# qinzheng93/GeoTransformer

Measured on NVIDIA H100. Metric: point-cloud pairs/sec (3DMatch-shape synth), higher is better.
Workload: dtype f32

## Files before the change

### geotransformer_b200/_lib.py

```python
import ctypes
import os
import threading

import torch

_HERE = os.path.dirname(os.path.abspath(__file__))
LIB_PATH = os.path.join(_HERE, 'libgeob200.so')
_lib = None

c_void_p, c_int64, c_int32, c_float, c_double, c_size_t, c_int = (
    ctypes.c_void_p, ctypes.c_int64, ctypes.c_int32, ctypes.c_float, ctypes.c_double, ctypes.c_size_t, ctypes.c_int)

SIGNATURES = {}


def _sig(name, restype, *argtypes):
    SIGNATURES[name] = (restype, list(argtypes))


P, I64, I32, F, D, SZ = c_void_p, c_int64, c_int32, c_float, c_double, c_size_t
_sig('geob200_last_error', ctypes.c_char_p)
_sig('geob200_launch_count', ctypes.c_uint64)
_sig('geob200_grid_subsample_workspace_bytes', SZ, I64, I64)
_sig('geob200_grid_subsample', c_int, P, I64, P, I64, F, P, P, P, SZ, P)
_sig('geob200_radius_search_workspace_bytes', SZ, I64, I64, I64)
_sig('geob200_radius_search', c_int, P, I64, P, I64, P, P, I64, F, I64, P, P, P, P, SZ, P)

_sig('geob200_neighbor_histogram', c_int, P, I64, I64, I64, I64, P, P)
_sig('geob200_kpconv_workspace_bytes', SZ, I64)
_sig('geob200_kpconv', c_int, P, P, P, P, I64, I64, I64, P, I64, P, P, I64, I64, F, P, P, SZ, P)
_sig('geob200_kpconv_tc_workspace_bytes', SZ, I64, I64, I64)
_sig('geob200_kpconv_tc', c_int, P, P, P, P, I64, I64, I64, P, I64, P, P, I64, I64, F, P, P, SZ, P)
_sig('geob200_set_linear_mode', None, c_int)
_sig('geob200_linear', c_int, P, I64, P, P, P, I64, I64, I64, I64, c_int, P)
_sig('geob200_split_tf32', c_int, P, I64, I64, I64, P, P)
_sig('geob200_linear_batched', c_int, P, I64, I64, P, I64, I64, P, I64, P, I64, I64, I64, I64, I64, I64, c_int, P)
_sig('geob200_group_norm_workspace_bytes', SZ, I64)
_sig('geob200_group_norm', c_int, P, I64, I64, I64, P, P, F, P, c_int, F, P, P, SZ, P)
_sig('geob200_fused_group_norm_workspace_bytes', SZ, I64, I64, I64)
_sig('geob200_linear_group_norm', c_int, P, I64, P, P, I64, I64, I64, I64, P, P, F, P, c_int, F, P, P, P, SZ, P)
_sig('geob200_kpconv_group_norm', c_int, P, P, P, P, I64, I64, I64, P, I64, P, P, I64, I64, F, I64, P, P, F, c_int, F, P, P, P, SZ,
     P, SZ, P)
_sig('geob200_group_norm_batched', c_int, P, I64, I64, I64, P, P, F, P, c_int, F, P, P, SZ, P, I64, P)
_sig('geob200_linear_group_norm_batched', c_int, P, I64, P, P, I64, I64, I64, I64, P, P, F, P, c_int, F, P, P, P, SZ, P, I64, P)
_sig('geob200_maxpool', c_int, P, P, I64, I64, I64, I64, P, P)
_sig('geob200_upsample_concat', c_int, P, P, I64, I64, P, I64, I64, I64, P, P)
_sig('geob200_point_to_node_partition_batched', c_int, P, P, I64, P, P, I64, P, P, P, P, P, P)
_sig('geob200_gather_rows', c_int, P, I64, I64, P, I64, P, P)
_sig('geob200_knn_partition', c_int, P, I64, P, I64, I64, P, P, P)
_sig('geob200_pairwise_distance', c_int, P, I64, P, I64, I64, c_int, P, P)
_sig('geob200_point_to_node_indices', c_int, P, I64, P, I64, P, P, P)
_sig('geob200_apply_transform', c_int, P, I64, P, P, P)
_sig('geob200_gse_indices_batched', c_int, P, I64, P, F, F, I64, P, P, P)
_sig('geob200_gse_embed_workspace_bytes', SZ, I64, I64)
_sig('geob200_gse_table_bytes', SZ, I64, I64, F, F)
_sig('geob200_gse_table_build', c_int, P, P, P, P, P, I64, I64, F, F, P, SZ, P)
_sig('geob200_gse_embed_table', c_int, P, P, I64, I64, P, SZ, I64, F, F, P, P, P, P, P, P, P)
_sig('geob200_gse_embed_pairs', c_int, P, P, I64, I64, P, P, P, P, P, P, P, P, c_int, P, SZ, P)
_sig('geob200_attention_workspace_bytes', SZ, I64, I64, I64)
_sig('geob200_attention', c_int, P, I64, P, I64, P, I64, P, P, P, I64, I64, I64, I64, P, I64, P, SZ, P)
_sig('geob200_set_attention_tma', c_int, c_int)
_sig('geob200_head_bias', c_int, P, I64, P, I64, I64, I64, P, P)
_sig('geob200_add_layernorm', c_int, P, P, P, P, I64, I64, F, P, P)
_sig('geob200_l2_normalize', c_int, P, I64, I64, P, P)
_sig('geob200_sinkhorn', c_int, P, P, P, P, I64, I64, I64, F, P, P)
# ... 128 lines not shown
```

### geotransformer_b200/csrc/kpconv.cu

```cuda
#include "common.cuh"
#include "geob200.h"

namespace geob200 {

constexpr int KP = 15;
constexpr int KP_PAD = 16;
constexpr int TQ = 32;
constexpr int CC = 32;

__device__ __forceinline__ void influence15(const float* __restrict__ kp_s, float rx, float ry, float rz, float inv_dummy,
                                            float sigma, float* w) {
#pragma unroll
    for (int k = 0; k < KP; ++k) {
        const float dx = rx - kp_s[3 * k], dy = ry - kp_s[3 * k + 1], dz = rz - kp_s[3 * k + 2];
        const float sq = __fadd_rn(__fadd_rn(__fmul_rn(dx, dx), __fmul_rn(dy, dy)), __fmul_rn(dz, dz));
        w[k] = fmaxf(1.0f - sqrtf(sq) / sigma, 0.0f);
    }
    (void)inv_dummy;
}

__global__ void __launch_bounds__(256) kpconv_c1_kernel(const float* __restrict__ feats, const float* __restrict__ q_pts,
                                                        const float* __restrict__ s_pts, const long long* __restrict__ nbr,
                                                        int H, const float* __restrict__ kp, const float* __restrict__ W,
                                                        const float* __restrict__ bias, float sigma, int Ns, int M, int Cout,
                                                        float* __restrict__ out) {
    __shared__ float kp_s[KP * 3];
    __shared__ float wk_s[16][KP_PAD];
    __shared__ float np_s[16];
    if (threadIdx.x < KP * 3) kp_s[threadIdx.x] = kp[threadIdx.x];
    __syncthreads();
    const int lane = threadIdx.x & 31, warp = threadIdx.x >> 5;
    const int sub = lane >> 4, sl = lane & 15;
    const int slot = warp * 2 + sub;
    const int m = blockIdx.x * 16 + slot;
    const bool live = m < M;
    float acc[KP];
#pragma unroll
    for (int k = 0; k < KP; ++k) acc[k] = 0.f;
    int npos = 0;
    if (live) {
        const float qx = q_pts[3ll * m], qy = q_pts[3ll * m + 1], qz = q_pts[3ll * m + 2];
        for (int h = sl; h < H; h += 16) {
            const long long idx = nbr[(long long)m * H + h];
            if (idx < Ns) {
                float w[KP];
                influence15(kp_s, s_pts[3 * idx] - qx, s_pts[3 * idx + 1] - qy, s_pts[3 * idx + 2] - qz, 0.f, sigma, w);
                const float f = feats[idx];
                npos += (f > 0.f);
#pragma unroll
                for (int k = 0; k < KP; ++k) acc[k] = fmaf(w[k], f, acc[k]);
// ... 4 lines not shown
    for (int k = 0; k < KP; ++k) {
#pragma unroll
        for (int o = 8; o > 0; o >>= 1) acc[k] += __shfl_xor_sync(0xffffffffu, acc[k], o);
    }
#pragma unroll
    for (int o = 8; o > 0; o >>= 1) npos += __shfl_xor_sync(0xffffffffu, npos, o);
    if (sl == 0) {
#pragma unroll
        for (int k = 0; k < KP; ++k) wk_s[slot][k] = acc[k];
        np_s[slot] = (float)max(npos, 1);
    }
    __syncwarp();
    if (!live) return;
    for (int c = sl; c < Cout; c += 16) {
        float o = 0.f;
#pragma unroll
        for (int k = 0; k < KP; ++k) o = fmaf(wk_s[slot][k], W[k * Cout + c], o);
        o = o / np_s[slot];
        if (bias != nullptr) o += bias[c];
        out[(long long)m * Cout + c] = o;
    }
}

__global__ void __launch_bounds__(256) row_positive_kernel(const float* __restrict__ x, int N, int C, unsigned char* __restrict__ pos) {
    const int lane = threadIdx.x & 31;
    const int n = blockIdx.x * 8 + (threadIdx.x >> 5);
    if (n >= N) return;
    float s = 0.f;
    for (int c = lane; c < C; c += 32) s += x[(long long)n * C + c];
    s = warp_sum(s);
    if (lane == 0) pos[n] = (s > 0.f) ? 1 : 0;
}

template <int CPL>
__global__ void __launch_bounds__(256, 4) kpconv_gather_kernel(const float* __restrict__ feats, const unsigned char* __restrict__ pos,
                                                            const float* __restrict__ q_pts, const float* __restrict__ s_pts,
                                                            const long long* __restrict__ nbr, int H, const float* __restrict__ kp,
                                                            float sigma, int Ns, int M, int Cin, float* __restrict__ wf,
                                                            float* __restrict__ inv_count) {
    __shared__ float infl[8][32][KP_PAD];
    __shared__ int sidx[8][32];
    __shared__ float kp_s[KP * 3];
    const int lane = threadIdx.x & 31, warp = threadIdx.x >> 5;
    if (threadIdx.x < KP * 3) kp_s[threadIdx.x] = kp[threadIdx.x];
    __syncthreads();
    const int m = blockIdx.x * 8 + warp;
    if (m >= M) return;
    const float qx = q_pts[3ll * m], qy = q_pts[3ll * m + 1], qz = q_pts[3ll * m + 2];
    int npos = 0;
    for (int c0 = 0; c0 < Cin; c0 += 32 * CPL) {
        float acc[CPL][KP];
#pragma unroll
        for (int p = 0; p < CPL; ++p)
#pragma unroll
            for (int k = 0; k < KP; ++k) acc[p][k] = 0.f;
        for (int h0 = 0; h0 < H; h0 += 32) {
            const int h = h0 + lane;
            const long long idx = (h < H) ? nbr[(long long)m * H + h] : (long long)Ns;
            float w[KP];
            int id = 0;
            if (idx < Ns) {
                id = (int)idx;
                influence15(kp_s, s_pts[3 * idx] - qx, s_pts[3 * idx + 1] - qy, s_pts[3 * idx + 2] - qz, 0.f, sigma, w);
                if (c0 == 0) npos += pos[idx];
            } else {
#pragma unroll
                for (int k = 0; k < KP; ++k) w[k] = 0.f;
            }
            __syncwarp();
#pragma unroll
            for (int k = 0; k < KP; ++k) infl[warp][lane][k] = w[k];
            infl[warp][lane][KP] = 0.f;
            sidx[warp][lane] = id;
            __syncwarp();
            const int hn = min(32, H - h0);
            for (int hb = 0; hb < hn; hb += 8) {
                float f[8][CPL];
#pragma unroll
                for (int u = 0; u < 8; ++u)
#pragma unroll
                    for (int p = 0; p < CPL; ++p)
                        f[u][p] = __ldg(feats + (long long)sidx[warp][(hb + u) & 31] * Cin + c0 + 32 * p + lane);
#pragma unroll
                for (int u = 0; u < 8; ++u) {
                    if (hb + u < hn) {
                        const float4* iv = reinterpret_cast<const float4*>(&infl[warp][hb + u][0]);
                        const float4 a0 = iv[0], a1 = iv[1], a2 = iv[2], a3 = iv[3];
                        const float wv[16] = {a0.x, a0.y, a0.z, a0.w, a1.x, a1.y, a1.z, a1.w, a2.x, a2.y, a2.z, a2.w, a3.x, a3.y, a3.z, a3.w};
#pragma unroll
                        for (int p = 0; p < CPL; ++p)
#pragma unroll
                            for (int k = 0; k < KP; ++k) acc[p][k] = fmaf(wv[k], f[u][p], acc[p][k]);
                    }
                }
            }
        }
#pragma unroll
        for (int p = 0; p < CPL; ++p) {
            float* wrow = wf + (long long)m * (KP * Cin) + c0 + 32 * p + lane;
#pragma unroll
            for (int k = 0; k < KP; ++k) wrow[(long long)k * Cin] = acc[p][k];
        }
    }
#pragma unroll
    for (int o = 16; o > 0; o >>= 1) npos += __shfl_xor_sync(0xffffffffu, npos, o);
    if (lane == 0) inv_count[m] = 1.0f / (float)max(npos, 1);
}

static void launch_kpconv_gather(const float* s_feats, const unsigned char* pos, const float* q_points, const float* s_points,
                                 const long long* neighbors, int n_neighbors, const float* kernel_points, float sigma, int n_support,
                                 int n_query, int c_in, float* wf, float* inv_count, cudaStream_t st) {
    const unsigned grid = (unsigned)((n_query + 7) / 8);
    if (c_in % 64 == 0)
        kpconv_gather_kernel<2><<<grid, 256, 0, st>>>(s_feats, pos, q_points, s_points, neighbors, n_neighbors, kernel_points, sigma,
                                                     n_support, n_query, c_in, wf, inv_count);
    else
        kpconv_gather_kernel<1><<<grid, 256, 0, st>>>(s_feats, pos, q_points, s_points, neighbors, n_neighbors, kernel_points, sigma,
                                                     n_support, n_query, c_in, wf, inv_count);
}

template <int RC>
__global__ void __launch_bounds__(256) kpconv_kernel(const float* __restrict__ feats, const unsigned char* __restrict__ pos,
                                                     const float* __restrict__ q_pts, const float* __restrict__ s_pts,
                                                     const long long* __restrict__ nbr, int H, const float* __restrict__ kp,
                                                     const float* __restrict__ W, const float* __restrict__ bias, float sigma,
                                                     int Ns, int M, int Cin, int Cout, float* __restrict__ out) {
    const int col0 = blockIdx.y * (RC * 32);
    extern __shared__ float smem[];
    float* wf = smem;
    float* infl = wf + TQ * KP * CC;
    int* sidx = (int*)(infl + 8 * 32 * KP_PAD);
    float* npos_s = (float*)(sidx + 8 * 32);
    float* kp_s = npos_s + TQ;
    const int lane = threadIdx.x & 31, warp = threadIdx.x >> 5;
    if (threadIdx.x < KP * 3) kp_s[threadIdx.x] = kp[threadIdx.x];
    __syncthreads();
    const int m0 = blockIdx.x * TQ;

    float acc_out[4][RC];
#pragma unroll
    for (int r = 0; r < 4; ++r)
#pragma unroll
        for (int j = 0; j < RC; ++j) acc_out[r][j] = 0.f;

    for (int c0 = 0; c0 < Cin; c0 += CC) {
        for (int q = warp; q < TQ; q += 8) {
            const int m = m0 + q;
            float acc[KP];
#pragma unroll
            for (int k = 0; k < KP; ++k) acc[k] = 0.f;
            int npos = 0;
// ... 594 lines not shown
            best = fmaxf(best, v);
        }
        y[(long long)m * C + c] = best;
    }
}

__global__ void __launch_bounds__(256) upsample_concat_kernel(const float* __restrict__ x, const long long* __restrict__ up,
                                                              int up_stride, int Ns, const float* __restrict__ skip, int M,
                                                              int C1, int C2, float* __restrict__ y) {
    const int lane = threadIdx.x & 31;
    const int m = blockIdx.x * 8 + (threadIdx.x >> 5);
    if (m >= M) return;
    const long long idx = up[(long long)m * up_stride];
    float* yr = y + (long long)m * (C1 + C2);
    for (int c = lane; c < C1; c += 32) yr[c] = (idx < Ns) ? x[idx * C1 + c] : 0.f;
    if (skip != nullptr)
        for (int c = lane; c < C2; c += 32) yr[C1 + c] = skip[(long long)m * C2 + c];
}

}

using namespace geob200;

namespace geob200 {
int linear_tc(const float* x, int64_t ldx, const float* w, int64_t ldw, const float* w_img, const float* bias, const float* row_scale, float* y, int64_t ldy,
              int64_t m, int64_t n, int64_t k, int relu, cudaStream_t st, const GnFuse* gn = nullptr);
static int g_linear_mode = 1;
}

extern "C" {

void geob200_set_linear_mode(int mode) { g_linear_mode = mode; }

size_t geob200_kpconv_workspace_bytes(int64_t n_support) { return (size_t)n_support + 256; }

size_t geob200_kpconv_tc_workspace_bytes(int64_t n_query, int64_t n_support, int64_t c_in) {
    return align_up((size_t)n_support, 256) + align_up((size_t)n_query * 4, 256) + (size_t)n_query * KP * (size_t)c_in * 4 + 1024;
}

int geob200_kpconv_tc(const float* s_feats, const float* q_points, const float* s_points, const int64_t* neighbors, int64_t n_query,
                      int64_t n_support, int64_t n_neighbors, const float* kernel_points, int64_t n_kernel, const float* weights_t,
                      const float* bias, int64_t c_in, int64_t c_out, float sigma, float* out, void* workspace, size_t workspace_bytes,
                      void* stream) {
    return geob200::kpconv_tc_impl(s_feats, q_points, s_points, neighbors, n_query, n_support, n_neighbors, kernel_points, n_kernel,
                                   weights_t, nullptr, bias, c_in, c_out, sigma, out, workspace, workspace_bytes, stream);
}
}

namespace geob200 {
int kpconv_tc_impl(const float* s_feats, const float* q_points, const float* s_points, const int64_t* neighbors, int64_t n_query,
                   int64_t n_support, int64_t n_neighbors, const float* kernel_points, int64_t n_kernel, const float* weights_t,
                   const float* w_img, const float* bias, int64_t c_in, int64_t c_out, float sigma, float* out, void* workspace,
                   size_t workspace_bytes, void* stream) {
    cudaStream_t st = (cudaStream_t)stream;
    GEOB_REQUIRE(n_kernel == KP, "kpconv_tc: kernel_size %lld unsupported", (long long)n_kernel);
    GEOB_REQUIRE(n_query > 0 && n_support > 0 && n_neighbors > 0, "kpconv_tc: empty input");
    GEOB_REQUIRE(c_in % 32 == 0 && c_out % 16 == 0 && c_out >= 32 && (c_out <= 128 || c_out % 128 == 0) && n_query >= 64,
                 "kpconv_tc: unsupported shape (%lld -> %lld, %lld queries)", (long long)c_in, (long long)c_out, (long long)n_query);
    GEOB_REQUIRE(workspace_bytes >= geob200_kpconv_tc_workspace_bytes(n_query, n_support, c_in), "kpconv_tc: workspace too small");
    Arena ar(workspace, workspace_bytes);
    unsigned char* pos = ar.take<unsigned char>(n_support);
    float* inv_count = ar.take<float>(n_query);
    float* wf = ar.take<float>((size_t)n_query * KP * c_in);
    row_positive_kernel<<<(unsigned)((n_support + 7) / 8), 256, 0, st>>>(s_feats, (int)n_support, (int)c_in, pos);
    launch_kpconv_gather(s_feats, pos, q_points, s_points, (const long long*)neighbors, (int)n_neighbors, kernel_points, sigma,
                         (int)n_support, (int)n_query, (int)c_in, wf, inv_count, st);
    GEOB_CHECK_LAUNCH();
    count_launches(2);
    const int rc = linear_tc(wf, KP * c_in, weights_t, KP * c_in, w_img, bias, inv_count, out, c_out, n_query, c_out, KP * c_in, 0, st);
    GEOB_REQUIRE(rc == 0, "kpconv_tc: tensor-core GEMM rejected the shape");
    return 0;
}

int linear_img(const float* x, int64_t ldx, const float* weight, const float* w_img, const float* bias, float* y, int64_t ldy,
               int64_t m, int64_t n, int64_t k, int relu, void* stream) {
    if (g_linear_mode == 1 && m > 0 && n > 0 && k > 0) {
        const int rc = linear_tc(x, ldx, weight, k, w_img, bias, nullptr, y, ldy, m, n, k, relu, (cudaStream_t)stream);
        if (rc <= 0) return rc;
    }
    return geob200_linear(x, ldx, weight, bias, y, ldy, m, n, k, relu, stream);
}
}

extern "C" {

int geob200_kpconv(const float* s_feats, const float* q_points, const float* s_points, const int64_t* neighbors,
                   int64_t n_query, int64_t n_support, int64_t n_neighbors, const float* kernel_points, int64_t n_kernel,
                   const float* weights, const float* bias, int64_t c_in, int64_t c_out, float sigma, float* out,
                   void* workspace, size_t workspace_bytes, void* stream) {
    cudaStream_t st = (cudaStream_t)stream;
    GEOB_REQUIRE(n_kernel == KP, "kpconv: kernel_size %lld unsupported (all shipped models use 15)", (long long)n_kernel);
    GEOB_REQUIRE(n_query > 0 && n_support > 0 && n_neighbors > 0, "kpconv: empty input");
    if (c_in == 1) {
        kpconv_c1_kernel<<<(unsigned)((n_query + 15) / 16), 256, 0, st>>>(s_feats, q_points, s_points, (const long long*)neighbors,
                                                                       (int)n_neighbors, kernel_points, weights, bias, sigma,
                                                                       (int)n_support, (int)n_query, (int)c_out, out);
        GEOB_CHECK_LAUNCH();
        count_launches(1);
        return 0;
// ... 231 lines not shown
                              const float* weights_t, const float* bias, int64_t c_in, int64_t c_out, float sigma, int64_t groups,
                              const float* gamma, const float* beta, float eps, int leaky, float slope, float* pre_norm, float* y,
                              void* gn_workspace, size_t gn_workspace_bytes, void* workspace, size_t workspace_bytes, void* stream) {
    return geob200::kpconv_group_norm_impl(s_feats, q_points, s_points, neighbors, n_query, n_support, n_neighbors, kernel_points, n_kernel,
                                           weights_t, bias, c_in, c_out, sigma, groups, gamma, beta, eps, leaky, slope, pre_norm, y,
                                           gn_workspace, gn_workspace_bytes, workspace, workspace_bytes, stream, nullptr);
}
}

namespace geob200 {
int kpconv_group_norm_impl(const float* s_feats, const float* q_points, const float* s_points, const int64_t* neighbors,
                           int64_t n_query, int64_t n_support, int64_t n_neighbors, const float* kernel_points, int64_t n_kernel,
                           const float* weights_t, const float* bias, int64_t c_in, int64_t c_out, float sigma, int64_t groups,
                           const float* gamma, const float* beta, float eps, int leaky, float slope, float* pre_norm, float* y,
                           void* gn_workspace, size_t gn_workspace_bytes, void* workspace, size_t workspace_bytes, void* stream,
                           const GnSeg* seg, const float* w_img) {
    cudaStream_t st = (cudaStream_t)stream;
    const int64_t np = (seg != nullptr && seg->n_pairs > 1) ? seg->n_pairs : 1;
    GEOB_REQUIRE(n_kernel == KP, "kpconv_group_norm: kernel_size %lld unsupported", (long long)n_kernel);
    GEOB_REQUIRE(n_query > 0 && n_support > 0 && n_neighbors > 0, "kpconv_group_norm: empty input");
    GEOB_REQUIRE(c_in % 32 == 0 && c_out % 16 == 0 && c_out >= 32 && (c_out <= 128 || c_out % 128 == 0) && n_query >= 64,
                 "kpconv_group_norm: unsupported shape (%lld -> %lld, %lld queries)", (long long)c_in, (long long)c_out,
                 (long long)n_query);
    GEOB_REQUIRE(groups > 0 && c_out % groups == 0, "kpconv_group_norm: bad group count");
    GEOB_REQUIRE(gn_workspace_bytes >= (np > 1 ? fused_group_norm_workspace_bytes_batched(n_query, c_out, groups, np)
                                               : geob200_fused_group_norm_workspace_bytes(n_query, c_out, groups)),
                 "kpconv_group_norm: GroupNorm workspace too small");
    GEOB_REQUIRE(workspace_bytes >= geob200_kpconv_tc_workspace_bytes(n_query, n_support, c_in), "kpconv_group_norm: workspace too small");
    Arena ar(workspace, workspace_bytes);
    unsigned char* pos = ar.take<unsigned char>(n_support);
    float* inv_count = ar.take<float>(n_query);
    float* wf = ar.take<float>((size_t)n_query * KP * c_in);
    row_positive_kernel<<<(unsigned)((n_support + 7) / 8), 256, 0, st>>>(s_feats, (int)n_support, (int)c_in, pos);
    launch_kpconv_gather(s_feats, pos, q_points, s_points, (const long long*)neighbors, (int)n_neighbors, kernel_points, sigma,
                         (int)n_support, (int)n_query, (int)c_in, wf, inv_count, st);
    GEOB_CHECK_LAUNCH();
    count_launches(2);
    const GnWs w = gn_carve(gn_workspace, gn_workspace_bytes, groups, np);
    GnFuse gn{(int)groups, 0, w.partial};
    int rc = linear_tc(wf, KP * c_in, weights_t, KP * c_in, w_img, bias, inv_count, pre_norm, c_out, n_query, c_out, KP * c_in, 0, st, &gn);
    if (rc < 0) return rc;
    if (rc == 0) {
        if (np > 1) {
            launch_gn_seg_apply(pre_norm, w, gamma, beta, nullptr, y, n_query, c_out, groups, eps, leaky, slope, *seg, st);
        } else {
            launch_gn_apply(pre_norm, w, gamma, beta, nullptr, y, n_query, c_out, groups, eps, leaky, slope, st);
            count_launches(2);
        }
        GEOB_CHECK_LAUNCH();
        return 0;
    }
    rc = linear_tc(wf, KP * c_in, weights_t, KP * c_in, w_img, bias, inv_count, pre_norm, c_out, n_query, c_out, KP * c_in, 0, st);
    GEOB_REQUIRE(rc == 0, "kpconv_group_norm: tensor-core GEMM rejected the shape");
    return group_norm_impl(pre_norm, n_query, c_out, groups, gamma, beta, eps, nullptr, leaky, slope, y, gn_workspace, gn_workspace_bytes,
                           stream, seg);
}
}

namespace geob200 {
static int make_seg(GnSeg* g, int64_t n_pairs, const int64_t* cloud_rows_h, int64_t n_rows) {
    GEOB_REQUIRE(n_pairs >= 1 && 2 * n_pairs <= GEOB_MAX_CLOUDS && cloud_rows_h != nullptr, "group_norm: 1 <= pairs per batch <= %d", GEOB_MAX_CLOUDS / 2);
    g->n_pairs = (int)n_pairs; g->n_clouds = (int)(2 * n_pairs); g->start[0] = 0;
    for (int c = 0; c < g->n_clouds; ++c) g->start[c + 1] = g->start[c] + (int)cloud_rows_h[c];
    GEOB_REQUIRE(g->start[g->n_clouds] == n_rows, "group_norm: cloud rows do not add up to n_rows");
    return 0;
}
}

// ... 46 lines not shown
```

### geotransformer_b200/functional.py

```python
import ctypes
import math

import torch

from . import _lib as L

_f32, _i64, _u8, _i32 = torch.float32, torch.int64, torch.uint8, torch.int32

GSE_MODE = int(__import__('os').environ.get('GEOB200_GSE_MODE', '5'))
GSE_TABLE_INV_STEP = int(__import__('os').environ.get('GEOB200_GSE_TABLE_INV_STEP', '256'))
GSE_TABLE_D_MAX = float(__import__('os').environ.get('GEOB200_GSE_TABLE_D_MAX', '96'))

EVENTS = None


class _timed:
    def __init__(self, name):
        self.name = name

    def __enter__(self):
        if EVENTS is not None:
            self.s = torch.cuda.Event(enable_timing=True)
            self.e = torch.cuda.Event(enable_timing=True)
            self.s.record()
# ... 31 lines not shown
    if ws is None or ws.numel() < need:
        ws = torch.zeros(max(int(need * 1.5), 1 << 20), dtype=_u8, device=device)
        _GN_WS[key] = ws
    return ws



KPCONV_MODE = 'tc'


def kpconv(s_feats, q_points, s_points, neighbor_indices, kernel_points, weights, bias, sigma, weights_t=None):
    s_feats, weights, bias = _detach(s_feats), _detach(weights), _detach(bias)
    _f(s_feats, 's_feats'); _f(q_points, 'q_points'); _f(s_points, 's_points')
    L.require_cuda(neighbor_indices, 'neighbor_indices', _i64)
    m, h = neighbor_indices.shape
    ns = s_points.shape[0]
    k, cin, cout = weights.shape
    out = torch.empty((m, cout), dtype=_f32, device=s_feats.device)
    lib = L.lib()
    if (KPCONV_MODE == 'tc' and cin % 32 == 0 and cout % 16 == 0 and cout >= 32 and (cout <= 128 or cout % 128 == 0) and m >= 64):
        if weights_t is None:
            weights_t = weights.reshape(k * cin, cout).t().contiguous()
        ws = L.workspace(lib.geob200_kpconv_tc_workspace_bytes(m, ns, cin), s_feats.device, 'kpconv_tc')
        L.check(lib.geob200_kpconv_tc(s_feats.data_ptr(), q_points.data_ptr(), s_points.data_ptr(), neighbor_indices.data_ptr(), m, ns,
                                      h, kernel_points.data_ptr(), k, weights_t.data_ptr(), L.ptr(bias), cin, cout, float(sigma),
                                      out.data_ptr(), ws.data_ptr(), ws.numel(), L.stream_ptr()), 'kpconv_tc')
        return out
    ws = L.workspace(lib.geob200_kpconv_workspace_bytes(ns), s_feats.device, 'kpconv')
    L.check(lib.geob200_kpconv(s_feats.data_ptr(), q_points.data_ptr(), s_points.data_ptr(),
                               neighbor_indices.data_ptr(), m, ns, h, kernel_points.data_ptr(), k,
                               weights.data_ptr(), L.ptr(bias), cin, cout, float(sigma), out.data_ptr(),
                               ws.data_ptr(), ws.numel(), L.stream_ptr()), 'kpconv')
    return out


def linear(x, weight, bias=None, relu=False, out=None):
    x, weight, bias = _detach(x), _detach(weight), _detach(bias)
    if not x.is_cuda or x.dtype != _f32 or x.stride(1) != 1:
        raise RuntimeError('linear: x must be a float32 CUDA tensor with unit inner stride')
    L.require_cuda(weight, 'weight', _f32)
    m, k = x.shape
    n = weight.shape[0]
    if out is None:
        out = torch.empty((m, n), dtype=_f32, device=x.device)
    L.check(L.lib().geob200_linear(x.data_ptr(), x.stride(0), weight.data_ptr(), L.ptr(bias), out.data_ptr(),
                                   out.stride(0), m, n, k, int(relu), L.stream_ptr()), 'linear')
    return out


def split_tf32(weight):
    weight = _detach(weight)
    if not weight.is_cuda or weight.dtype != _f32 or weight.dim() != 2 or weight.stride(1) != 1:
        raise RuntimeError('split_tf32: weight must be a 2-D float32 CUDA tensor with unit inner stride')
    n, k = weight.shape
    out = torch.empty((2 * n, k), dtype=_f32, device=weight.device)
    L.check(L.lib().geob200_split_tf32(weight.data_ptr(), weight.stride(0), n, k, out.data_ptr(), L.stream_ptr()), 'split_tf32')
    return out


def group_norm(x, weight, bias, groups, eps=1e-5, negative_slope=None, residual=None):
    x, weight, bias = _detach(x), _detach(weight), _detach(bias)
    _f(x, 'x')
    n, c = x.shape
    ws = _gn_workspace(x.device, groups)
    y = torch.empty_like(x)
    L.check(L.lib().geob200_group_norm(x.data_ptr(), n, c, groups, weight.data_ptr(), bias.data_ptr(), float(eps),
# ... 1260 lines not shown
```

### geotransformer_b200/synth.py

```python
import numpy as np


def _room(rng, n, L, sigma, off):
    face = rng.integers(0, 3, size=n)
    uv = rng.uniform(0.0, L, size=(n, 2))
    pts = np.zeros((n, 3), dtype=np.float64)
    for f in range(3):
        m = face == f
        axes = [a for a in range(3) if a != f]
        pts[m, axes[0]] = uv[m, 0]
        pts[m, axes[1]] = uv[m, 1]
    pts += rng.normal(0.0, sigma, size=(n, 3))
    return pts + off


def _sphere(rng, n, R, sigma):
    v = rng.normal(size=(n, 3))
    v /= np.linalg.norm(v, axis=1, keepdims=True)
    return v * R + rng.normal(0.0, sigma, size=(n, 3))


def _ground(rng, n, R, sigma):
    r = R * np.sqrt(rng.uniform(size=n))
    th = rng.uniform(0.0, 2 * np.pi, size=n)
# ... 11 lines not shown

WORKLOADS = {
    'demo2k': ('3dmatch', _room, dict(n=2048, L=0.90, sigma=0.003, off=0.1), 1.0),
    'modelnet717': ('modelnet', _sphere, dict(n=717, R=0.60, sigma=0.01), 1.0),
    '3dmatch20k': ('3dmatch', _room, dict(n=20000, L=1.85, sigma=0.003, off=0.1), 1.0),
    'kitti60k': ('kitti', _ground, dict(n=60000, R=60.0, sigma=0.05), 10.0),
    'kitti20k': ('kitti', _ground, dict(n=20000, R=35.0, sigma=0.05), 10.0),
    'kitti4k': ('kitti', _ground, dict(n=4000, R=18.0, sigma=0.05), 10.0),
}


def make_pair(workload, index=0, base_seed=7351):
    cfg_name, gen, kw, tscale = WORKLOADS[workload]
    rng = np.random.default_rng(base_seed + index)
    ref = gen(rng, **kw)
    world = gen(rng, **kw)
    axis = rng.normal(size=3)
    angle = rng.uniform(0.0, np.pi / 4)
    R = _rodrigues(axis, angle)
    t = rng.uniform(-0.5, 0.5, size=3) * tscale
    src = (world - t) @ R
    T = np.eye(4)
    T[:3, :3] = R
    T[:3, 3] = t
    n = ref.shape[0]
    return {
        'ref_points': ref.astype(np.float32),
        'src_points': src.astype(np.float32),
        'ref_feats': np.ones((n, 1), dtype=np.float32),
        'src_feats': np.ones((n, 1), dtype=np.float32),
        'transform': T.astype(np.float32),
        'config': cfg_name,
    }
```

### include/geob200.h

```cpp
#ifndef GEOB200_H
#define GEOB200_H

#include <stddef.h>
#include <stdint.h>

#ifdef __cplusplus
extern "C" {
#endif

const char* geob200_last_error(void);
uint64_t geob200_launch_count(void);


size_t geob200_grid_subsample_workspace_bytes(int64_t n_points, int64_t batch);
int geob200_grid_subsample(const float* points, int64_t n_points, const int64_t* lengths_h, int64_t batch, float voxel,
                           float* s_points, int64_t* s_lengths, void* workspace, size_t workspace_bytes, void* stream);

size_t geob200_radius_search_workspace_bytes(int64_t n_query, int64_t n_support, int64_t batch);
int geob200_radius_search(const float* q_points, int64_t n_query, const float* s_points, int64_t n_support,
                          const int64_t* q_lengths_h, const int64_t* s_lengths_h, int64_t batch, float radius,
                          int64_t width, int64_t* out, int32_t* counts, int32_t* max_count, void* workspace,
                          size_t workspace_bytes, void* stream);

int geob200_neighbor_histogram(const int64_t* neighbors, int64_t n_rows, int64_t width, int64_t n_support, int64_t hist_n,
                               int32_t* hist, void* stream);


size_t geob200_kpconv_workspace_bytes(int64_t n_support);
int geob200_kpconv(const float* s_feats, const float* q_points, const float* s_points, const int64_t* neighbors,
                   int64_t n_query, int64_t n_support, int64_t n_neighbors, const float* kernel_points, int64_t n_kernel,
                   const float* weights, const float* bias, int64_t c_in, int64_t c_out, float sigma, float* out,
                   void* workspace, size_t workspace_bytes, void* stream);

size_t geob200_kpconv_tc_workspace_bytes(int64_t n_query, int64_t n_support, int64_t c_in);
int geob200_kpconv_tc(const float* s_feats, const float* q_points, const float* s_points, const int64_t* neighbors, int64_t n_query,
                      int64_t n_support, int64_t n_neighbors, const float* kernel_points, int64_t n_kernel, const float* weights_t,
                      const float* bias, int64_t c_in, int64_t c_out, float sigma, float* out, void* workspace, size_t workspace_bytes,
                      void* stream);

int geob200_split_tf32(const float* w, int64_t ld, int64_t n, int64_t k, float* out, void* stream);

void geob200_set_linear_mode(int mode);
int geob200_linear(const float* x, int64_t ldx, const float* weight, const float* bias, float* y, int64_t ldy, int64_t m,
                   int64_t n, int64_t k, int relu, void* stream);
int geob200_linear_batched(const float* x, int64_t ldx, int64_t stride_x, const float* weight, int64_t ldw, int64_t stride_w,
                           const float* bias, int64_t stride_b, float* y, int64_t ldy, int64_t stride_y, int64_t m, int64_t n,
                           int64_t k, int64_t batch, int relu, void* stream);

size_t geob200_group_norm_workspace_bytes(int64_t groups);
int geob200_group_norm(const float* x, int64_t n_rows, int64_t channels, int64_t groups, const float* gamma,
                       const float* beta, float eps, const float* residual, int leaky, float slope, float* y,
                       void* workspace, size_t workspace_bytes, void* stream);

size_t geob200_fused_group_norm_workspace_bytes(int64_t n_rows, int64_t channels, int64_t groups);
int geob200_linear_group_norm(const float* x, int64_t ldx, const float* weight, const float* bias, int64_t m, int64_t n, int64_t k,
                              int64_t groups, const float* gamma, const float* beta, float eps, const float* residual, int leaky,
                              float slope, float* pre_norm, float* y, void* workspace, size_t workspace_bytes, void* stream);
int geob200_kpconv_group_norm(const float* s_feats, const float* q_points, const float* s_points, const int64_t* neighbors,
                              int64_t n_query, int64_t n_support, int64_t n_neighbors, const float* kernel_points, int64_t n_kernel,
                              const float* weights_t, const float* bias, int64_t c_in, int64_t c_out, float sigma, int64_t groups,
                              const float* gamma, const float* beta, float eps, int leaky, float slope, float* pre_norm, float* y,
                              void* gn_workspace, size_t gn_workspace_bytes, void* workspace, size_t workspace_bytes, void* stream);

int geob200_group_norm_batched(const float* x, int64_t n_rows, int64_t channels, int64_t groups, const float* gamma, const float* beta,
                               float eps, const float* residual, int leaky, float slope, float* y, void* workspace, size_t workspace_bytes,
                               void* stream, int64_t n_pairs, const int64_t* cloud_rows_h);
int geob200_linear_group_norm_batched(const float* x, int64_t ldx, const float* weight, const float* bias, int64_t m, int64_t n, int64_t k,
                                      int64_t groups, const float* gamma, const float* beta, float eps, const float* residual, int leaky,
                                      float slope, float* pre_norm, float* y, void* workspace, size_t workspace_bytes, void* stream,
                                      int64_t n_pairs, const int64_t* cloud_rows_h);

// ... 251 lines not shown
```

Baseline: 360.7.

## Add block-cooperative float4 KPConv gather kernel and trim padded neighbor slots

Adds a new gather kernel for c_in >= 128. It stages neighbor indices and kernel-point influences for several queries in shared memory at block level, then has each thread accumulate four channels using float4 loads and streaming stores. For the narrow-channel path it also uses a warp ballot to skip padded neighbor slots and batches of eight that hold no live entries. It exposes a standalone gather entry point and a mode switch, and adds a helper that records layer inputs. This targets wasted loads on padding and poor memory coalescing in the weighted-feature gather, at the cost of more shared memory and lower occupancy.

```diff
diff --git a/geotransformer_b200/_lib.py b/geotransformer_b200/_lib.py
--- a/geotransformer_b200/_lib.py
+++ b/geotransformer_b200/_lib.py
@@ -31,6 +31,8 @@
 _sig('geob200_kpconv', c_int, P, P, P, P, I64, I64, I64, P, I64, P, P, I64, I64, F, P, P, SZ, P)
 _sig('geob200_kpconv_tc_workspace_bytes', SZ, I64, I64, I64)
 _sig('geob200_kpconv_tc', c_int, P, P, P, P, I64, I64, I64, P, I64, P, P, I64, I64, F, P, P, SZ, P)
+_sig('geob200_kpconv_gather', c_int, P, P, P, P, I64, I64, I64, P, I64, I64, F, P, P, P, P)
+_sig('geob200_set_kpconv_gather', c_int, c_int)
 _sig('geob200_set_linear_mode', None, c_int)
 _sig('geob200_linear', c_int, P, I64, P, P, P, I64, I64, I64, I64, c_int, P)
 _sig('geob200_split_tf32', c_int, P, I64, I64, I64, P, P)
diff --git a/geotransformer_b200/csrc/kpconv.cu b/geotransformer_b200/csrc/kpconv.cu
--- a/geotransformer_b200/csrc/kpconv.cu
+++ b/geotransformer_b200/csrc/kpconv.cu
@@ -8,14 +8,16 @@
 constexpr int TQ = 32;
 constexpr int CC = 32;
 
+__device__ __forceinline__ float influence1(const float* __restrict__ kp_s, int k, float rx, float ry, float rz, float sigma) {
+    const float dx = rx - kp_s[3 * k], dy = ry - kp_s[3 * k + 1], dz = rz - kp_s[3 * k + 2];
+    const float sq = __fadd_rn(__fadd_rn(__fmul_rn(dx, dx), __fmul_rn(dy, dy)), __fmul_rn(dz, dz));
+    return fmaxf(1.0f - sqrtf(sq) / sigma, 0.0f);
+}
+
 __device__ __forceinline__ void influence15(const float* __restrict__ kp_s, float rx, float ry, float rz, float inv_dummy,
                                             float sigma, float* w) {
 #pragma unroll
-    for (int k = 0; k < KP; ++k) {
-        const float dx = rx - kp_s[3 * k], dy = ry - kp_s[3 * k + 1], dz = rz - kp_s[3 * k + 2];
-        const float sq = __fadd_rn(__fadd_rn(__fmul_rn(dx, dx), __fmul_rn(dy, dy)), __fmul_rn(dz, dz));
-        w[k] = fmaxf(1.0f - sqrtf(sq) / sigma, 0.0f);
-    }
+    for (int k = 0; k < KP; ++k) w[k] = influence1(kp_s, k, rx, ry, rz, sigma);
     (void)inv_dummy;
 }
 
@@ -86,7 +88,7 @@
     if (lane == 0) pos[n] = (s > 0.f) ? 1 : 0;
 }
 
-template <int CPL>
+template <int CPL, bool TRIM>
 __global__ void __launch_bounds__(256, 4) kpconv_gather_kernel(const float* __restrict__ feats, const unsigned char* __restrict__ pos,
                                                             const float* __restrict__ q_pts, const float* __restrict__ s_pts,
                                                             const long long* __restrict__ nbr, int H, const float* __restrict__ kp,
@@ -127,17 +129,20 @@
             infl[warp][lane][KP] = 0.f;
             sidx[warp][lane] = id;
             __syncwarp();
-            const int hn = min(32, H - h0);
+            const unsigned live = TRIM ? __ballot_sync(0xffffffffu, idx < Ns) : 0xffffffffu;
+            const int hn = TRIM ? 32 - __clz(live) : min(32, H - h0);
             for (int hb = 0; hb < hn; hb += 8) {
+                if (TRIM && ((live >> hb) & 0xffu) == 0) continue;
                 float f[8][CPL];
 #pragma unroll
                 for (int u = 0; u < 8; ++u)
 #pragma unroll
                     for (int p = 0; p < CPL; ++p)
-                        f[u][p] = __ldg(feats + (long long)sidx[warp][(hb + u) & 31] * Cin + c0 + 32 * p + lane);
+                        f[u][p] = (!TRIM || ((live >> ((hb + u) & 31)) & 1u))
+                                      ? __ldg(feats + (long long)sidx[warp][(hb + u) & 31] * Cin + c0 + 32 * p + lane) : 0.f;
 #pragma unroll
                 for (int u = 0; u < 8; ++u) {
-                    if (hb + u < hn) {
+                    if (TRIM ? ((live >> ((hb + u) & 31)) & 1u) != 0 : hb + u < hn) {
                         const float4* iv = reinterpret_cast<const float4*>(&infl[warp][hb + u][0]);
                         const float4 a0 = iv[0], a1 = iv[1], a2 = iv[2], a3 = iv[3];
                         const float wv[16] = {a0.x, a0.y, a0.z, a0.w, a1.x, a1.y, a1.z, a1.w, a2.x, a2.y, a2.z, a2.w, a3.x, a3.y, a3.z, a3.w};
@@ -153,24 +158,130 @@
         for (int p = 0; p < CPL; ++p) {
             float* wrow = wf + (long long)m * (KP * Cin) + c0 + 32 * p + lane;
 #pragma unroll
-            for (int k = 0; k < KP; ++k) wrow[(long long)k * Cin] = acc[p][k];
+            for (int k = 0; k < KP; ++k) {
+                if (TRIM) __stcs(wrow + (long long)k * Cin, acc[p][k]);
+                else wrow[(long long)k * Cin] = acc[p][k];
+            }
         }
     }
 #pragma unroll
     for (int o = 16; o > 0; o >>= 1) npos += __shfl_xor_sync(0xffffffffu, npos, o);
     if (lane == 0) inv_count[m] = 1.0f / (float)max(npos, 1);
 }
+
+constexpr int GT_THREADS = 256;
+constexpr int GT_ROWS = 512;
+constexpr int GT_U = 8;
+constexpr int GT_QMAX = 32;
+
+__global__ void __launch_bounds__(GT_THREADS, 2) kpconv_gather4_kernel(const float* __restrict__ feats, const unsigned char* __restrict__ pos,
+                                                                      const float* __restrict__ q_pts, const float* __restrict__ s_pts,
+                                                                      const long long* __restrict__ nbr, int H, const float* __restrict__ kp,
+                                                                      float sigma, int Ns, int M, int Cin, int L, float* __restrict__ wf,
+                                                                      float* __restrict__ inv_count) {
+    __shared__ __align__(16) float infl[GT_ROWS * KP_PAD + GT_QMAX * 4];
+    __shared__ int sidx[GT_ROWS];
+    __shared__ float kp_s[KP * 3];
+    __shared__ int npos_s[GT_QMAX];
+    const int tid = threadIdx.x;
+    const int QC = GT_THREADS / L, HT = GT_ROWS / QC, qstride = HT * KP_PAD + 4;
+    if (tid < KP * 3) kp_s[tid] = kp[tid];
+    if (tid < GT_QMAX) npos_s[tid] = 0;
+    const long long m0 = (long long)blockIdx.x * QC;
+    const int uq = tid / L, ul = tid - uq * L;
+    const long long um = m0 + uq;
+    const bool ulive = uq < QC && um < M;
+    for (int c0 = 0; c0 < Cin; c0 += 4 * L) {
+        const int c = c0 + 4 * ul;
+        const bool cl = ulive && c < Cin;
+        const float* fcol = feats + c;
+        float acc[KP][4];
+#pragma unroll
+        for (int k = 0; k < KP; ++k) acc[k][0] = acc[k][1] = acc[k][2] = acc[k][3] = 0.f;
+        for (int h0 = 0; h0 < H; h0 += HT) {
+            __syncthreads();
+#pragma unroll 1
+            for (int r = tid; r < GT_ROWS; r += GT_THREADS) {
+                const int iq = r / HT, h = h0 + (r - iq * HT);
+                const long long im = m0 + iq;
+                int id = -1;
+                if (iq < QC && im < M && h < H) {
+                    const long long idx = nbr[im * H + h];
+                    if (idx < Ns) {
+                        id = (int)idx;
+                        const float rx = s_pts[3 * idx] - q_pts[3 * im], ry = s_pts[3 * idx + 1] - q_pts[3 * im + 1];
+                        const float rz = s_pts[3 * idx + 2] - q_pts[3 * im + 2];
+                        float* row = infl + iq * qstride + (r - iq * HT) * KP_PAD;
+#pragma unroll 5
+                        for (int k = 0; k < KP; ++k) row[k] = influence1(kp_s, k, rx, ry, rz, sigma);
+                        row[KP] = 0.f;
+                        if (c0 == 0 && pos[idx]) atomicAdd(&npos_s[iq], 1);
+                    }
+                }
+                sidx[r] = id;
+            }
+            __syncthreads();
+            if (cl) {
+                const int hn = min(HT, H - h0);
+                const int* ts = sidx + uq * HT;
+                const float* ti = infl + uq * qstride;
+                for (int j0 = 0; j0 < hn; j0 += GT_U) {
+                    int id[GT_U];
+                    float4 f[GT_U];
+#pragma unroll
+                    for (int u = 0; u < GT_U; ++u) id[u] = (j0 + u < hn) ? ts[j0 + u] : -1;
+#pragma unroll
+                    for (int u = 0; u < GT_U; ++u)
+                        if (id[u] >= 0) f[u] = __ldg(reinterpret_cast<const float4*>(fcol + (long long)id[u] * Cin));
+#pragma unroll
+                    for (int u = 0; u < GT_U; ++u) {
+                        if (id[u] >= 0) {
+                            const float4* iv = reinterpret_cast<const float4*>(ti + (j0 + u) * KP_PAD);
+                            const float4 a0 = iv[0], a1 = iv[1], a2 = iv[2], a3 = iv[3];
+                            const float wv[KP] = {a0.x, a0.y, a0.z, a0.w, a1.x, a1.y, a1.z, a1.w, a2.x, a2.y, a2.z, a2.w, a3.x, a3.y, a3.z};
+#pragma unroll
+                            for (int k = 0; k < KP; ++k) {
+                                acc[k][0] = fmaf(wv[k], f[u].x, acc[k][0]);
+                                acc[k][1] = fmaf(wv[k], f[u].y, acc[k][1]);
+                                acc[k][2] = fmaf(wv[k], f[u].z, acc[k][2]);
+                                acc[k][3] = fmaf(wv[k], f[u].w, acc[k][3]);
+                            }
+                        }
+                    }
+                }
+            }
+        }
+        if (cl) {
+            float* wrow = wf + um * (KP * (long long)Cin) + c;
+#pragma unroll
+            for (int k = 0; k < KP; ++k)
+                __stcs(reinterpret_cast<float4*>(wrow + (long long)k * Cin), make_float4(acc[k][0], acc[k][1], acc[k][2], acc[k][3]));
+        }
+    }
+    __syncthreads();
+    if (tid < QC && m0 + tid < M) inv_count[m0 + tid] = 1.0f / (float)max(npos_s[tid], 1);
+}
+
+static int g_gather_mode = 1;
 
 static void launch_kpconv_gather(const float* s_feats, const unsigned char* pos, const float* q_points, const float* s_points,
                                  const long long* neighbors, int n_neighbors, const float* kernel_points, float sigma, int n_support,
                                  int n_query, int c_in, float* wf, float* inv_count, cudaStream_t st) {
+    const bool use4 = g_gather_mode == 2 || (g_gather_mode == 1 && c_in >= 128);
+    if (use4 && (((uintptr_t)s_feats | (uintptr_t)wf) & 15) == 0) {
+        const int L = min(c_in / 4, GT_THREADS), qc = GT_THREADS / L;
+        kpconv_gather4_kernel<<<(unsigned)((n_query + qc - 1) / qc), GT_THREADS, 0, st>>>(
+            s_feats, pos, q_points, s_points, neighbors, n_neighbors, kernel_points, sigma, n_support, n_query, c_in, L, wf, inv_count);
+        return;
+    }
     const unsigned grid = (unsigned)((n_query + 7) / 8);
-    if (c_in % 64 == 0)
-        kpconv_gather_kernel<2><<<grid, 256, 0, st>>>(s_feats, pos, q_points, s_points, neighbors, n_neighbors, kernel_points, sigma,
-                                                     n_support, n_query, c_in, wf, inv_count);
-    else
-        kpconv_gather_kernel<1><<<grid, 256, 0, st>>>(s_feats, pos, q_points, s_points, neighbors, n_neighbors, kernel_points, sigma,
-                                                     n_support, n_query, c_in, wf, inv_count);
+#define LAUNCH_GATHER(CPLV, TRIMV)                                                                                              \
+    kpconv_gather_kernel<CPLV, TRIMV><<<grid, 256, 0, st>>>(s_feats, pos, q_points, s_points, neighbors, n_neighbors, kernel_points, \
+                                                           sigma, n_support, n_query, c_in, wf, inv_count)
+    if (c_in % 64 == 0) LAUNCH_GATHER(2, false);
+    else if (g_gather_mode != 0) LAUNCH_GATHER(1, true);
+    else LAUNCH_GATHER(1, false);
+#undef LAUNCH_GATHER
 }
 
 template <int RC>
@@ -843,6 +954,30 @@
                       void* stream) {
     return geob200::kpconv_tc_impl(s_feats, q_points, s_points, neighbors, n_query, n_support, n_neighbors, kernel_points, n_kernel,
                                    weights_t, nullptr, bias, c_in, c_out, sigma, out, workspace, workspace_bytes, stream);
+}
+
+int geob200_kpconv_gather(const float* s_feats, const float* q_points, const float* s_points, const int64_t* neighbors, int64_t n_query,
+                          int64_t n_support, int64_t n_neighbors, const float* kernel_points, int64_t n_kernel, int64_t c_in, float sigma,
+                          uint8_t* pos, float* wf, float* inv_count, void* stream) {
+    cudaStream_t st = (cudaStream_t)stream;
+    GEOB_REQUIRE(n_kernel == KP, "kpconv_gather: kernel_size %lld unsupported", (long long)n_kernel);
+    GEOB_REQUIRE(n_query > 0 && n_support > 0 && n_neighbors > 0, "kpconv_gather: empty input");
+    GEOB_REQUIRE(c_in % 32 == 0 && n_query < (1ll << 31) && n_support < (1ll << 31) && n_neighbors < (1ll << 31),
+                 "kpconv_gather: unsupported shape (c_in %lld)", (long long)c_in);
+    GEOB_REQUIRE(pos != nullptr && wf != nullptr && inv_count != nullptr && ((uintptr_t)wf & 15) == 0 && ((uintptr_t)s_feats & 15) == 0,
+                 "kpconv_gather: outputs missing or wf / s_feats not 16-byte aligned");
+    row_positive_kernel<<<(unsigned)((n_support + 7) / 8), 256, 0, st>>>(s_feats, (int)n_support, (int)c_in, pos);
+    launch_kpconv_gather(s_feats, pos, q_points, s_points, (const long long*)neighbors, (int)n_neighbors, kernel_points, sigma,
+                         (int)n_support, (int)n_query, (int)c_in, wf, inv_count, st);
+    GEOB_CHECK_LAUNCH();
+    count_launches(2);
+    return 0;
+}
+
+int geob200_set_kpconv_gather(int mode) {
+    GEOB_REQUIRE(mode >= 0 && mode <= 2, "set_kpconv_gather: mode %d not in 0..2", mode);
+    g_gather_mode = mode;
+    return 0;
 }
 }
 
diff --git a/geotransformer_b200/functional.py b/geotransformer_b200/functional.py
--- a/geotransformer_b200/functional.py
+++ b/geotransformer_b200/functional.py
@@ -87,6 +87,21 @@
                                weights.data_ptr(), L.ptr(bias), cin, cout, float(sigma), out.data_ptr(),
                                ws.data_ptr(), ws.numel(), L.stream_ptr()), 'kpconv')
     return out
+
+
+def kpconv_gather(s_feats, q_points, s_points, neighbor_indices, kernel_points, sigma):
+    _f(s_feats, 's_feats'); _f(q_points, 'q_points'); _f(s_points, 's_points')
+    L.require_cuda(neighbor_indices, 'neighbor_indices', _i64)
+    m, h = neighbor_indices.shape
+    ns, cin = s_feats.shape
+    dev = s_feats.device
+    pos = torch.empty(ns, dtype=torch.uint8, device=dev)
+    wf = torch.empty((m, kernel_points.shape[0] * cin), dtype=_f32, device=dev)
+    inv_count = torch.empty(m, dtype=_f32, device=dev)
+    L.check(L.lib().geob200_kpconv_gather(s_feats.data_ptr(), q_points.data_ptr(), s_points.data_ptr(), neighbor_indices.data_ptr(), m,
+                                          ns, h, kernel_points.data_ptr(), kernel_points.shape[0], cin, float(sigma), pos.data_ptr(),
+                                          wf.data_ptr(), inv_count.data_ptr(), L.stream_ptr()), 'kpconv_gather')
+    return wf, inv_count
 
 
 def linear(x, weight, bias=None, relu=False, out=None):
diff --git a/geotransformer_b200/synth.py b/geotransformer_b200/synth.py
--- a/geotransformer_b200/synth.py
+++ b/geotransformer_b200/synth.py
@@ -67,3 +67,39 @@
         'transform': T.astype(np.float32),
         'config': cfg_name,
     }
+
+
+def kpconv_gather_inputs(model, cfg, workload, n_pairs, device='cuda'):
+    import torch
+    from . import functional as GF
+    from .utils.data import registration_collate_fn_stack_mode
+    keys = ('ref_points', 'src_points', 'ref_feats', 'src_feats', 'transform')
+    pairs = [{k: make_pair(workload, i)[k] for k in keys} for i in range(n_pairs)]
+    b = cfg.backbone
+    limits = cfg.neighbor_limits or [27, 75, 147, 157, 119][:b.num_stages]
+    data = registration_collate_fn_stack_mode(pairs, b.num_stages, b.init_voxel_size, b.init_radius, limits, device=device)
+    layers = []
+
+    def record(s_feats, q_points, s_points, neighbors, kernel_points, sigma):
+        if s_feats.shape[1] % 32 == 0:
+            layers.append({'s_feats': s_feats.detach().clone(), 'q_points': q_points, 's_points': s_points, 'neighbors': neighbors,
+                           'kernel_points': kernel_points.detach(), 'sigma': float(sigma)})
+
+    plain, fused = GF.kpconv, GF.kpconv_group_norm
+
+    def kpconv(s_feats, q_points, s_points, neighbors, kernel_points, weights, bias, sigma, *a, **kw):
+        record(s_feats, q_points, s_points, neighbors, kernel_points, sigma)
+        return plain(s_feats, q_points, s_points, neighbors, kernel_points, weights, bias, sigma, *a, **kw)
+
+    def kpconv_group_norm(s_feats, q_points, s_points, neighbors, kernel_points, weights, bias, sigma, *a, **kw):
+        record(s_feats, q_points, s_points, neighbors, kernel_points, sigma)
+        return fused(s_feats, q_points, s_points, neighbors, kernel_points, weights, bias, sigma, *a, **kw)
+
+    GF.kpconv, GF.kpconv_group_norm = kpconv, kpconv_group_norm
+    try:
+        with torch.no_grad():
+            model.backbone(data['features'], data)
+        torch.cuda.synchronize()
+    finally:
+        GF.kpconv, GF.kpconv_group_norm = plain, fused
+    return layers
diff --git a/include/geob200.h b/include/geob200.h
--- a/include/geob200.h
+++ b/include/geob200.h
@@ -37,6 +37,10 @@
                       int64_t n_support, int64_t n_neighbors, const float* kernel_points, int64_t n_kernel, const float* weights_t,
                       const float* bias, int64_t c_in, int64_t c_out, float sigma, float* out, void* workspace, size_t workspace_bytes,
                       void* stream);
+int geob200_kpconv_gather(const float* s_feats, const float* q_points, const float* s_points, const int64_t* neighbors, int64_t n_query,
+                          int64_t n_support, int64_t n_neighbors, const float* kernel_points, int64_t n_kernel, int64_t c_in, float sigma,
+                          uint8_t* pos, float* wf, float* inv_count, void* stream);
+int geob200_set_kpconv_gather(int mode);
 
 int geob200_split_tf32(const float* w, int64_t ld, int64_t n, int64_t k, float* out, void* stream);
 
```

Result: faster. 368.1, median of 6 (+2.0%).

## Add shared-memory row-cached KPConv gather kernel with block-wide influence precompute

Applied to the files above, without the earlier changes.

Adds a new KPConv gather kernel that, for a block of 8 queries, stages neighbor indices, relative positions and all 15 kernel-point influence weights in shared memory. Each warp then accumulates weighted features with float2 loads and splits the 15 kernel points across half-warps. Results are written with streaming stores. The aim is to avoid recomputing influences per channel chunk and to improve load vectorisation in the gather stage before the TF32 GEMM. It uses dynamic shared memory sized by neighbor count, which can lower occupancy. It only applies when c_in is a multiple of 128, the shared memory fits, and the features are 8-byte aligned; a runtime toggle is added to fall back to the old kernel.

```diff
diff --git a/geotransformer_b200/_lib.py b/geotransformer_b200/_lib.py
--- a/geotransformer_b200/_lib.py
+++ b/geotransformer_b200/_lib.py
@@ -31,6 +31,7 @@
 _sig('geob200_kpconv', c_int, P, P, P, P, I64, I64, I64, P, I64, P, P, I64, I64, F, P, P, SZ, P)
 _sig('geob200_kpconv_tc_workspace_bytes', SZ, I64, I64, I64)
 _sig('geob200_kpconv_tc', c_int, P, P, P, P, I64, I64, I64, P, I64, P, P, I64, I64, F, P, P, SZ, P)
+_sig('geob200_set_kpconv_gather', c_int, c_int)
 _sig('geob200_set_linear_mode', None, c_int)
 _sig('geob200_linear', c_int, P, I64, P, P, P, I64, I64, I64, I64, c_int, P)
 _sig('geob200_split_tf32', c_int, P, I64, I64, I64, P, P)
diff --git a/geotransformer_b200/csrc/kpconv.cu b/geotransformer_b200/csrc/kpconv.cu
--- a/geotransformer_b200/csrc/kpconv.cu
+++ b/geotransformer_b200/csrc/kpconv.cu
@@ -161,9 +161,115 @@
     if (lane == 0) inv_count[m] = 1.0f / (float)max(npos, 1);
 }
 
-static void launch_kpconv_gather(const float* s_feats, const unsigned char* pos, const float* q_points, const float* s_points,
-                                 const long long* neighbors, int n_neighbors, const float* kernel_points, float sigma, int n_support,
-                                 int n_query, int c_in, float* wf, float* inv_count, cudaStream_t st) {
+constexpr int GQ = 8;
+constexpr size_t GATHER_ROW_SMEM = KP_PAD * 4 + 16 + 4;
+constexpr size_t GATHER_MAX_SMEM = 227 * 1024;
+__global__ void __launch_bounds__(256, 3) kpconv_gather_rows_kernel(
+    const float* __restrict__ feats, const unsigned char* __restrict__ pos, const float* __restrict__ q_pts,
+    const float* __restrict__ s_pts, const long long* __restrict__ nbr, int H, const float* __restrict__ kp, float sigma, int Ns,
+    int M, int Cin, float* __restrict__ wf, float* __restrict__ inv_count) {
+    constexpr int NC = 2;
+    constexpr int U = 8 / NC;
+    extern __shared__ float4 gsm[];
+    float4* infl = gsm;
+    float4* rel = infl + GQ * H * 4;
+    int* sidx = reinterpret_cast<int*>(rel + GQ * H);
+    const int t = threadIdx.x, lane = t & 31, warp = t >> 5;
+    const int m0 = blockIdx.x * GQ;
+    const int R = min(GQ, M - m0) * H;
+    for (int r = t; r < R; r += 256) {
+        const long long idx = nbr[(long long)m0 * H + r];
+        float4 d = make_float4(0.f, 0.f, 0.f, 0.f);
+        int id = 0;
+        if (idx < Ns) {
+            const long long m = m0 + r / H;
+            id = (int)idx;
+            d = make_float4(s_pts[3 * idx] - q_pts[3 * m], s_pts[3 * idx + 1] - q_pts[3 * m + 1], s_pts[3 * idx + 2] - q_pts[3 * m + 2], 1.f);
+        }
+        rel[r] = d;
+        sidx[r] = id;
+    }
+    __syncthreads();
+    {
+        const int k = t & 15;
+        float kx = 0.f, ky = 0.f, kz = 0.f;
+        if (k < KP) { kx = kp[3 * k]; ky = kp[3 * k + 1]; kz = kp[3 * k + 2]; }
+        float* iw = reinterpret_cast<float*>(infl);
+        for (int r = t >> 4; r < R; r += 16) {
+            const float4 d = rel[r];
+            float w = 0.f;
+            if (k < KP && d.w != 0.f) {
+                const float dx = d.x - kx, dy = d.y - ky, dz = d.z - kz;
+                const float sq = __fadd_rn(__fadd_rn(__fmul_rn(dx, dx), __fmul_rn(dy, dy)), __fmul_rn(dz, dz));
+                w = fmaxf(1.0f - sqrtf(sq) / sigma, 0.0f);
+            }
+            iw[r * 16 + k] = w;
+        }
+    }
+    __syncthreads();
+    const int m = m0 + warp;
+    if (m >= M) return;
+    const float4* iq = infl + warp * H * 4 + (lane >> 4) * 2;
+    const int* qidx = sidx + warp * H;
+    int npos = 0;
+    for (int h = lane; h < H; h += 32)
+        if (rel[warp * H + h].w != 0.f) npos += pos[qidx[h]];
+#pragma unroll
+    for (int o = 16; o > 0; o >>= 1) npos += __shfl_xor_sync(0xffffffffu, npos, o);
+    if (lane == 0) inv_count[m] = 1.0f / (float)max(npos, 1);
+    const int k0 = (lane >> 4) * 8, cl = 2 * (lane & 15);
+    for (int c0 = 0; c0 < Cin; c0 += 32 * NC) {
+        float acc[NC][2][8];
+#pragma unroll
+        for (int p = 0; p < NC; ++p)
+#pragma unroll
+            for (int j = 0; j < 8; ++j) acc[p][0][j] = acc[p][1][j] = 0.f;
+        const float* fb = feats + c0 + cl;
+        for (int h0 = 0; h0 < H; h0 += U) {
+            float2 f[U][NC];
+#pragma unroll
+            for (int u = 0; u < U; ++u) {
+                const long long id = qidx[min(h0 + u, H - 1)];
+#pragma unroll
+                for (int p = 0; p < NC; ++p) f[u][p] = __ldg(reinterpret_cast<const float2*>(fb + id * Cin + 32 * p));
+            }
+#pragma unroll
+            for (int u = 0; u < U; ++u) {
+                if (h0 + u < H) {
+                    const float4 a = iq[(h0 + u) * 4], b = iq[(h0 + u) * 4 + 1];
+                    const float wv[8] = {a.x, a.y, a.z, a.w, b.x, b.y, b.z, b.w};
+#pragma unroll
+                    for (int p = 0; p < NC; ++p)
+#pragma unroll
+                        for (int j = 0; j < 8; ++j) {
+                            acc[p][0][j] = fmaf(wv[j], f[u][p].x, acc[p][0][j]);
+                            acc[p][1][j] = fmaf(wv[j], f[u][p].y, acc[p][1][j]);
+                        }
+                }
+            }
+        }
+        float* wrow = wf + (long long)m * (KP * Cin) + (long long)k0 * Cin + c0 + cl;
+#pragma unroll
+        for (int j = 0; j < 8; ++j)
+            if (k0 + j < KP)
+#pragma unroll
+                for (int p = 0; p < NC; ++p)
+                    __stcs(reinterpret_cast<float2*>(wrow + (long long)j * Cin + 32 * p), make_float2(acc[p][0][j], acc[p][1][j]));
+    }
+}
+
+static bool g_gather_rows = true;
+
+static int launch_kpconv_gather(const float* s_feats, const unsigned char* pos, const float* q_points, const float* s_points,
+                                const long long* neighbors, int n_neighbors, const float* kernel_points, float sigma, int n_support,
+                                int n_query, int c_in, float* wf, float* inv_count, cudaStream_t st) {
+    const size_t smem = (size_t)GQ * n_neighbors * GATHER_ROW_SMEM;
+    if (g_gather_rows && c_in % 128 == 0 && smem <= GATHER_MAX_SMEM && (reinterpret_cast<uintptr_t>(s_feats) & 7) == 0) {
+        if (smem > 48 * 1024 && ensure_max_smem((const void*)kpconv_gather_rows_kernel)) return -1;
+        kpconv_gather_rows_kernel<<<(unsigned)((n_query + GQ - 1) / GQ), 256, smem, st>>>(
+            s_feats, pos, q_points, s_points, neighbors, n_neighbors, kernel_points, sigma, n_support, n_query, c_in, wf, inv_count);
+        return 0;
+    }
     const unsigned grid = (unsigned)((n_query + 7) / 8);
     if (c_in % 64 == 0)
         kpconv_gather_kernel<2><<<grid, 256, 0, st>>>(s_feats, pos, q_points, s_points, neighbors, n_neighbors, kernel_points, sigma,
@@ -171,6 +277,7 @@
     else
         kpconv_gather_kernel<1><<<grid, 256, 0, st>>>(s_feats, pos, q_points, s_points, neighbors, n_neighbors, kernel_points, sigma,
                                                      n_support, n_query, c_in, wf, inv_count);
+    return 0;
 }
 
 template <int RC>
@@ -831,6 +938,12 @@
 
 void geob200_set_linear_mode(int mode) { g_linear_mode = mode; }
 
+int geob200_set_kpconv_gather(int mode) {
+    GEOB_REQUIRE(mode == 0 || mode == 1, "set_kpconv_gather: mode must be 0 or 1, got %d", mode);
+    g_gather_rows = mode == 1;
+    return 0;
+}
+
 size_t geob200_kpconv_workspace_bytes(int64_t n_support) { return (size_t)n_support + 256; }
 
 size_t geob200_kpconv_tc_workspace_bytes(int64_t n_query, int64_t n_support, int64_t c_in) {
@@ -862,8 +975,9 @@
     float* inv_count = ar.take<float>(n_query);
     float* wf = ar.take<float>((size_t)n_query * KP * c_in);
     row_positive_kernel<<<(unsigned)((n_support + 7) / 8), 256, 0, st>>>(s_feats, (int)n_support, (int)c_in, pos);
-    launch_kpconv_gather(s_feats, pos, q_points, s_points, (const long long*)neighbors, (int)n_neighbors, kernel_points, sigma,
-                         (int)n_support, (int)n_query, (int)c_in, wf, inv_count, st);
+    if (launch_kpconv_gather(s_feats, pos, q_points, s_points, (const long long*)neighbors, (int)n_neighbors, kernel_points, sigma,
+                             (int)n_support, (int)n_query, (int)c_in, wf, inv_count, st))
+        return -1;
     GEOB_CHECK_LAUNCH();
     count_launches(2);
     const int rc = linear_tc(wf, KP * c_in, weights_t, KP * c_in, w_img, bias, inv_count, out, c_out, n_query, c_out, KP * c_in, 0, st);
@@ -1161,8 +1275,9 @@
     float* inv_count = ar.take<float>(n_query);
     float* wf = ar.take<float>((size_t)n_query * KP * c_in);
     row_positive_kernel<<<(unsigned)((n_support + 7) / 8), 256, 0, st>>>(s_feats, (int)n_support, (int)c_in, pos);
-    launch_kpconv_gather(s_feats, pos, q_points, s_points, (const long long*)neighbors, (int)n_neighbors, kernel_points, sigma,
-                         (int)n_support, (int)n_query, (int)c_in, wf, inv_count, st);
+    if (launch_kpconv_gather(s_feats, pos, q_points, s_points, (const long long*)neighbors, (int)n_neighbors, kernel_points, sigma,
+                             (int)n_support, (int)n_query, (int)c_in, wf, inv_count, st))
+        return -1;
     GEOB_CHECK_LAUNCH();
     count_launches(2);
     const GnWs w = gn_carve(gn_workspace, gn_workspace_bytes, groups, np);
diff --git a/include/geob200.h b/include/geob200.h
--- a/include/geob200.h
+++ b/include/geob200.h
@@ -37,6 +37,7 @@
                       int64_t n_support, int64_t n_neighbors, const float* kernel_points, int64_t n_kernel, const float* weights_t,
                       const float* bias, int64_t c_in, int64_t c_out, float sigma, float* out, void* workspace, size_t workspace_bytes,
                       void* stream);
+int geob200_set_kpconv_gather(int mode);
 
 int geob200_split_tf32(const float* w, int64_t ld, int64_t n, int64_t k, float* out, void* stream);
 
```

After: 436.5 before, 441.4 after, median of 6. No clear change (+1.1%).
